# kessel/dune-pnp

Hardware: AMD Instinct MI355X
Metric: assembled DOFs/s + BiCGStab iters/s, 3-species PNP on pore.msh-refined (higher is better)
Workload: dtype f64; 1 GPU; config 3: stationary 3-ion PNP, test/pore_pnp/pore.msh refined k=4 x 1 mirrored copies; dofs=2214099, dofs_per_gpu=2214099, mesh_vertices=738033, triangles=1470464, parallelism=mesh partition (RCB) x1, preconditioner=ilu0, colors=4, sell_slots=5176768, blocks=5155025

## Files before the change

### dune-pnp_amd/csrc/assemble.hip

```cpp
#include <cstdlib>

#include <hip/hip_ext.h>

#include "element.h"
#include "kernels.h"

namespace pnp {

namespace {

template <int OP, int KC = 0>
__device__ __forceinline__ void store_block(double *__restrict__ vc, int lane, int s,
                                            const double *Kc) {
  constexpr int NK = OpTraits<OP>::NK;
  static_assert(!KC || OP == OP_PNP, "constant planes: the PNP operator only");
  constexpr int Q0 = KC ? 2 : 0;
#ifdef ASM_STORE_PLAIN
  store_vals<NK, Q0>(vc + size_t(s) * NK * kRows, lane, Kc);
#else
  store_vals_nt<NK, Q0>(vc + size_t(s) * NK * kRows, lane, Kc);
#endif
}

template <int NF>
// ... 136 lines not shown
      for (int v = 0; v < NK; v++) F[v] += P[v];
      store_block<OP>(vc, lane, 1, F);
    }
    store_block<OP>(vc, lane, 0, D);
  }
  residual_tail<NF>(a, row, a.rowflag[row], R);
}

#ifndef ASM_SU
#define ASM_SU 4
#endif
template <int OP>
__host__ __device__ constexpr int asm_lds_rec() {
  return 2 + OpTraits<OP>::NF + (OP == OP_DIFF || OP == OP_DIFF_IE || OP == OP_POISSON) +
         (OP == OP_POISSON);
}
template <int OP>
constexpr int asm_kc() {
  return OP == OP_PNP;
}
constexpr int kPipeDw = 11;
template <class P>
__device__ __forceinline__ void lds_dma4(const P *src, uint32_t *dst_wave) {
  __builtin_amdgcn_global_load_lds(
      (const __attribute__((address_space(1))) void *)(src),
      (__attribute__((address_space(3))) void *)(dst_wave), 4, 0, 0);
}
__device__ __forceinline__ int const_ld(const int *p, int i) {
  return ((const __attribute__((address_space(4))) int *)(p))[i];
}
__device__ __forceinline__ int row_block_const(const DevLayout &L, int b, int nwg) {
  return L.blkmap ? const_ld(L.blkmap, xcd_block(b, nwg, 1)) : xcd_block(b, nwg, L.xcd_remap);
}
template <int OP, int JAC, int MINW, int FANR, int SPLIT = FANR, int STAGE = 0, int LDSG = 0,
          int KC = 0, int PIPE = 0>
__global__ __launch_bounds__(256, MINW) void k_assemble_ga(DevLayout L, AsmArgs a) {
  using T = OpTraits<OP>;
  constexpr int NF = T::NF, NK = T::NK, NS = FANR;
  constexpr bool AUX0 = OP == OP_DIFF || OP == OP_DIFF_IE || OP == OP_POISSON;
  constexpr bool AUX1 = OP == OP_POISSON;
  constexpr int RW = asm_lds_rec<OP>();
  static_assert(!PIPE || (JAC && FANR == 9 && !STAGE && !LDSG), "PIPE: the direct Jacobian walk");
  extern __shared__ double srec[];
  __shared__ uint32_t pfb[PIPE ? 4 * kPipeDw * kRows : 1];
  const int ntiles = (L.n_owned + 255) / 256, G = gridDim.x;
  const int wv = PIPE ? __builtin_amdgcn_readfirstlane(int(threadIdx.x) / kRows) : 0;
  const int ln = int(threadIdx.x) % kRows;
  uint32_t *const pw = pfb + (PIPE ? wv * kPipeDw * kRows : 0);
  int tile = blockIdx.x, b0 = -1, b1 = -1, b2 = -1, o0 = 0, o1 = 0, c1 = 0;
  auto tile_blk = [&](int t) { return t < ntiles ? row_block_const(L, t, ntiles) : -1; };
  auto wave_chunk = [&](int b) {
    return (b >= 0 && b * 256 + wv * kRows < L.n_owned) ? b * 4 + wv : -1;
  };
  auto prefetch = [&](int b, int off, int clen) {
    if (wave_chunk(b) < 0) return;
    const int r0 = b * 256 + wv * kRows;
    const int *cix = L.colidx + off + ln;
#pragma unroll
    for (int k = 1; k < NS; k++)
      lds_dma4(cix + (k < clen ? k : 0) * kRows, pw + (k - 1) * kRows);
    const uint32_t *m =
        reinterpret_cast<const uint32_t *>(L.rowmeta + min(r0 + ln, L.n_owned - 1));
    lds_dma4(m, pw + 8 * kRows);
    lds_dma4(m + 1, pw + 9 * kRows);
    lds_dma4(reinterpret_cast<const uint32_t *>(a.rowflag + r0) + (ln >> 2), pw + 10 * kRows);
  };
  if constexpr (PIPE) {
    if (tile >= ntiles) return;
    b0 = tile_blk(tile);
    b1 = tile_blk(tile + G);
    b2 = tile_blk(tile + 2 * G);
    int c0 = 0;
    if (wave_chunk(b0) >= 0) {
      o0 = const_ld(L.chunk_off, wave_chunk(b0));
      c0 = const_ld(L.chunk_len, wave_chunk(b0));
    }
    if (wave_chunk(b1) >= 0) {
      o1 = const_ld(L.chunk_off, wave_chunk(b1));
      c1 = const_ld(L.chunk_len, wave_chunk(b1));
    }
    prefetch(b0, o0, c0);
  }
  int o2 = 0, c2 = 0, b3 = -1;
  const auto advance = [&]() {
    tile += G;
    b0 = b1, o0 = o1;
    b1 = b2, o1 = o2, c1 = c2;
    b2 = b3;
    return b0 >= 0;
  };
  do {
    const int blk = PIPE ? b0 : row_block(L, blockIdx.x, gridDim.x);
    const int row0 = blk * blockDim.x + threadIdx.x;
    const bool live = row0 < L.n_owned;
    if (!PIPE && !LDSG && !live) return;
    const int row = live ? row0 : 0;
    const int chunk = row / kRows, lane = row % kRows;
    int cj[NS];
    uint64_t meta_pf = 0;
    unsigned fl_pf = 0;
    if constexpr (PIPE) {
      asm volatile("s_waitcnt vmcnt(0)" ::: "memory");
#pragma unroll
      for (int k = 1; k < NS; k++) cj[k] = int(pw[(k - 1) * kRows + ln]);
      meta_pf = uint64_t(pw[8 * kRows + ln]) | (uint64_t(pw[9 * kRows + ln]) << 32);
      fl_pf = (pw[10 * kRows + ln] >> (8 * (ln & 3))) & 0xffu;
      asm volatile("s_waitcnt lgkmcnt(0)" ::: "memory");
      prefetch(b1, o1, c1);
      o2 = c2 = 0;
      if (wave_chunk(b2) >= 0) {
        o2 = const_ld(L.chunk_off, wave_chunk(b2));
        c2 = const_ld(L.chunk_len, wave_chunk(b2));
      }
      b3 = tile_blk(tile + 3 * G);
      if (!live) continue;
    }
    const int off = PIPE ? o0 : L.chunk_off[chunk];
    const uint64_t meta = PIPE ? meta_pf : L.rowmeta[row];
    const int len = int(meta & 63);
    const bool closed = (meta >> 6) & 1;
    const unsigned brk = unsigned(meta >> 8);
    double *__restrict__ vc = a.vals + size_t(off) * NK;

    if constexpr (PIPE) {
    } else if constexpr (LDSG) {
      const uint16_t *__restrict__ lix = L.lidx + off + lane;
#pragma unroll
      for (int k = 1; k < NS; k++) {
        const int t = lix[(k < len ? k : 0) * kRows];
        cj[k] = k < len ? t : 0;
// ... 125 lines not shown
          double Ct[NK];
#pragma unroll
          for (int v = 0; v < NK; v++) Ct[v] = 0;
          element<OP, JAC, KC>(a, G, pi2.y, pn[s].y, pt.y, ui, un[s], ut, ai, a0[s], at0, aq,
                               a1[s], at1, R, D, P, Ct);
          if constexpr (JAC) {
            if (s == 1 && closed) {
#pragma unroll
              for (int v = 0; v < NK; v++) F[v] = P[v];
            } else {
              put(s, P);
            }
#pragma unroll
            for (int v = 0; v < NK; v++) P[v] = Ct[v];
          }
        } else if constexpr (JAC) {
          put(s, P);
#pragma unroll
          for (int v = 0; v < NK; v++) P[v] = 0;
        }
      }
    }
    if constexpr (JAC) {
      if (closed) {
#pragma unroll
        for (int v = 0; v < NK; v++) F[v] += P[v];
        store_block<OP, KC>(vc, lane, 1, F);
      }
      store_block<OP, KC>(vc, lane, 0, D);
    }
    residual_tail<NF>(a, row, PIPE ? fl_pf : unsigned(a.rowflag[row]), R);
  } while (PIPE && advance());
}

template <int OP>
__global__ __launch_bounds__(256) void k_mass_apply(DevLayout L, double tau, double pi, int cyl,
                                                    const double *__restrict__ xo,
                                                    double *__restrict__ cvec) {
  constexpr int NF = OpTraits<OP>::NF;
  const int row = blockIdx.x * blockDim.x + threadIdx.x;
  if (row >= L.n_owned) return;
  const int chunk = row / kRows, lane = row % kRows;
  const int off = L.chunk_off[chunk];
  const uint64_t meta = L.rowmeta[row];
  const int len = int(meta & 63);
  const bool closed = (meta >> 6) & 1;
  const int *cix = L.colidx + off + lane;
  const double2 pi2 = reinterpret_cast<const double2 *>(L.xy)[row];
  double acc = 0;
  for (int s = 1; s < len; ++s) {
    const int t = (s + 1 < len) ? s + 1 : (closed ? 1 : -1);
    if (t < 0 || ((meta >> (8 + s)) & 1)) continue;
    const int b = cix[s * kRows], c = cix[t * kRows];
    const double2 pb2 = reinterpret_cast<const double2 *>(L.xy)[b];
    const double2 pc2 = reinterpret_cast<const double2 *>(L.xy)[c];
    Geo G;
    geometry(pi2.x, pi2.y, pb2.x, pb2.y, pc2.x, pc2.y, G);
    if constexpr (OP == OP_PNP_IE) {
      double Mii, Mib, Mic;
      mass_q2(G, cyl, pi, pi2.y, pb2.y, pc2.y, Mii, Mib, Mic);
      acc += tau * ((xo[size_t(row) * 3 + 1] + xo[size_t(row) * 3 + 2]) * Mii +
                    (xo[size_t(b) * 3 + 1] + xo[size_t(b) * 3 + 2]) * Mib +
                    (xo[size_t(c) * 3 + 1] + xo[size_t(c) * 3 + 2]) * Mic);
    } else {
      acc += xo[row] * G.adet * (1.0 / 12.0) + (xo[b] + xo[c]) * G.adet * (1.0 / 24.0);
    }
// ... 23 lines not shown
                 uo = x[size_t(q.z) * 3 + f];
    gf[f][0] = ua * G.gi0 + uc * G.gb0 + uo * G.gc0;
    gf[f][1] = ua * G.gi1 + uc * G.gb1 + uo * G.gc1;
  }
  const double cp = 0.5 * (x[size_t(q.x) * 3 + 1] + x[size_t(q.y) * 3 + 1]);
  const double cm = 0.5 * (x[size_t(q.x) * 3 + 2] + x[size_t(q.y) * 3 + 2]);
  const double tx = pc.x - pa.x, ty = pc.y - pa.y;
  const double len = sqrt(tx * tx + ty * ty);
  double factor = len;
  if (cyl) factor *= 2 * pi * (0.5 * (pa.y + pc.y));
  double nx = ty / len, ny = -tx / len;
  if (nx * (po.x - pa.x) + ny * (po.y - pa.y) > 0) {
    nx = -nx;
    ny = -ny;
  }
  const double gp0 = factor * gf[0][0] * cp, gp1 = factor * gf[0][1] * cp;
  out[2 * size_t(k)] = (-factor * gf[1][0] + gp0) * nx + (-factor * gf[1][1] + gp1) * ny;
  const double r = cm / cp;
  out[2 * size_t(k) + 1] =
      (-factor * gf[2][0] - gp0 * r) * nx + (-factor * gf[2][1] - gp1 * r) * ny;
}

}

hipError_t launch_ion_flux(int ns, const int4 *seg, const double *xy, const double *x, int cyl,
                           double pi, double *out, hipStream_t s) {
  if (ns == 0) return hipSuccess;
  hipLaunchKernelGGL(k_ion_flux, dim3((ns + 255) / 256), dim3(256), 0, s, ns, seg, xy, x, cyl, pi,
                     out);
  return hipGetLastError();
}

constexpr bool kAsmPipeDefault = false;

template <int OP>
static int launch_pipe(const DevLayout &L, const AsmArgs &a, int cap, hipStream_t s, hipEvent_t t0,
                       hipEvent_t t1) {
  if constexpr (asm_kc<OP>()) {
    const auto kern = k_assemble_ga<OP, 1, 3, 9, 6, 0, 0, 1, 1>;
    static const int resident = [&] {
      int dev = 0, cus = 0, per_cu = 0;
      if (hipGetDevice(&dev) != hipSuccess ||
          hipDeviceGetAttribute(&cus, hipDeviceAttributeMultiprocessorCount, dev) != hipSuccess ||
          hipOccupancyMaxActiveBlocksPerMultiprocessor(&per_cu, kern, 256, 0) != hipSuccess)
        return 0;
      return per_cu * cus;
    }();
    const int ntiles = (L.n_owned + 255) / 256;
    int g = resident >= 8 ? resident / 8 * 8 : 8;
    if (g > ntiles) g = ntiles;
    if (cap > 0 && g > cap) g = cap;
    hipExtLaunchKernelGGL(kern, dim3(g), dim3(256), 0, s, t0, t1, 0, L, a);
    return 1;
  } else {
    return 0;
  }
}

hipError_t launch_assemble(const DevLayout &L, const AsmArgs &a, hipStream_t s, hipEvent_t t0,
                           hipEvent_t t1, int *pipelined) {
  if (pipelined) *pipelined = 0;
  if (L.n_owned == 0) return hipSuccess;
  dim3 grid((L.n_owned + 255) / 256), block(256);
  static const int waves = [] {
    const char *e = getenv("PNP_ASM_WAVES");
    return (e && atoi(e) == 4) ? 4 : 3;
  }();
  static const bool fanr_ok = [] {
    const char *e = getenv("PNP_ASM_FANR");
    return !(e && atoi(e) == 0);
  }();
  static const int ga = [] {
    const char *e = getenv("PNP_ASM_GA");
    return e ? atoi(e) : 4;
  }();
  const int fanr = !fanr_ok ? 0 : (L.max_slots <= 9 ? 9 : (L.max_slots <= 12 ? 12 : 0));
  static const int lds_env = [] {
    const char *e = getenv("PNP_ASM_LDS");
    return e ? (atoi(e) == 1 ? 1 : 0) : -1;
  }();
  static const bool cold_hint = [] {
    const char *e = getenv("PNP_ASM_COLD_HINT");
    return !(e && e[0] == '0');
  }();
  const auto lds_walk = [&](int nk) {
    return lds_env == 1 ||
           (lds_env < 0 && (size_t(L.n_owned) * 7 * size_t(nk) * 8 > (size_t(512) << 20) ||
                            (cold_hint && a.cold)));
  };
  static const bool pipe_on = [] {
    const char *e = getenv("PNP_ASM_PIPE");
    return e ? atoi(e) != 0 : kAsmPipeDefault;
  }();
  static const int pipe_cap = [] {
    const char *e = getenv("PNP_ASM_PIPE_GRID");
    return (e && atoi(e) >= 1) ? atoi(e) : 0;
  }();
  int piped = 0;
#define PNP_ASM_CASE(OPK)                                                          \
  case OPK:                                                                        \
    if (!fanr && a.jac)                                                            \
      hipExtLaunchKernelGGL((k_assemble<OPK, 1, 3, 0>), grid, block, 0, s, t0, t1, 0, L, a);     \
    else if (!fanr)                                                                \
      hipExtLaunchKernelGGL((k_assemble<OPK, 0, 4, 0>), grid, block, 0, s, t0, t1, 0, L, a);     \
    else if (!a.jac && fanr == 9 && ga && lds_env == 1 && L.uown &&                 \
             size_t(L.unmax) * asm_lds_rec<OPK>() * 8 <= 53 * 1024)                    \
      hipExtLaunchKernelGGL((k_assemble_ga<OPK, 0, 3, 9, 9, 0, 1>), grid, block,         \
                         size_t(L.unmax) * asm_lds_rec<OPK>() * 8, s, t0, t1, 0, L, a);             \
    else if (!a.jac && fanr == 9 && ga)                                            \
      hipExtLaunchKernelGGL((k_assemble_ga<OPK, 0, 3, 9>), grid, block, 0, s, t0, t1, 0, L, a);  \
    else if (!a.jac)                                                               \
      hipExtLaunchKernelGGL((k_assemble<OPK, 0, 4, 12>), grid, block, 0, s, t0, t1, 0, L, a);    \
    else if (ga == 1 && fanr == 9)                                                 \
      hipExtLaunchKernelGGL((k_assemble_ga<OPK, 1, 3, 9>), grid, block, 0, s, t0, t1, 0, L, a);  \
    else if (ga == 2 && fanr == 9)                                                 \
      hipExtLaunchKernelGGL((k_assemble_ga<OPK, 1, 2, 9>), grid, block, 0, s, t0, t1, 0, L, a);  \
    else if (ga == 3 && fanr == 9)                                                 \
      hipExtLaunchKernelGGL((k_assemble_ga<OPK, 1, 3, 9, 5>), grid, block, 0, s, t0, t1, 0, L, a); \
    else if (ga == 4 && fanr == 9 && asm_kc<OPK>() && a.kconst &&                   \
             lds_walk(OpTraits<OPK>::NK) && L.uown &&                               \
             size_t(L.unmax) * asm_lds_rec<OPK>() * 8 <= 53 * 1024)                    \
      hipExtLaunchKernelGGL((k_assemble_ga<OPK, 1, 3, 9, 6, 0, 1, asm_kc<OPK>()>), grid,  \
                         block, size_t(L.unmax) * asm_lds_rec<OPK>() * 8, s, t0, t1, 0, L, a); \
    else if (ga == 4 && fanr == 9 && asm_kc<OPK>() && a.kconst && pipe_on)         \
      piped = launch_pipe<OPK>(L, a, pipe_cap, s, t0, t1);                         \
    else if (ga == 4 && fanr == 9 && asm_kc<OPK>() && a.kconst)                    \
      hipExtLaunchKernelGGL((k_assemble_ga<OPK, 1, 3, 9, 6, 0, 0, asm_kc<OPK>()>), grid,  \
                         block, 0, s, t0, t1, 0, L, a);                             \
    else if (ga == 4 && fanr == 9 && lds_walk(OpTraits<OPK>::NK) && L.uown &&       \
             size_t(L.unmax) * asm_lds_rec<OPK>() * 8 <= 53 * 1024)                    \
      hipExtLaunchKernelGGL((k_assemble_ga<OPK, 1, 3, 9, 6, 0, 1>), grid, block,         \
                         size_t(L.unmax) * asm_lds_rec<OPK>() * 8, s, t0, t1, 0, L, a);             \
    else if (ga == 4 && fanr == 9)                                                 \
      hipExtLaunchKernelGGL((k_assemble_ga<OPK, 1, 3, 9, 6>), grid, block, 0, s, t0, t1, 0, L, a); \
    else if (ga == 5 && fanr == 9)                                                 \
      hipExtLaunchKernelGGL((k_assemble_ga<OPK, 1, 3, 9, 3>), grid, block, 0, s, t0, t1, 0, L, a); \
    else if (ga == 6 && fanr == 9)                                                 \
      hipExtLaunchKernelGGL((k_assemble_ga<OPK, 1, 3, 9, 6, 1>), grid, block, 0, s, t0, t1, 0, L, a); \
    else if (fanr == 12)                                                           \
      hipExtLaunchKernelGGL((k_assemble<OPK, 1, 3, 12>), grid, block, 0, s, t0, t1, 0, L, a);    \
    else if (waves == 3)                                                           \
      hipExtLaunchKernelGGL((k_assemble<OPK, 1, 3, 9>), grid, block, 0, s, t0, t1, 0, L, a);     \
    else                                                                           \
      hipExtLaunchKernelGGL((k_assemble<OPK, 1, 4, 9>), grid, block, 0, s, t0, t1, 0, L, a);     \
    break;
  switch (a.kind) {
    PNP_ASM_CASE(OP_PNP)
    PNP_ASM_CASE(OP_PNP_IE)
    PNP_ASM_CASE(OP_PB)
    PNP_ASM_CASE(OP_DIFF)
    PNP_ASM_CASE(OP_DIFF_IE)
    PNP_ASM_CASE(OP_POISSON)
  default:
    return hipErrorInvalidValue;
  }
#undef PNP_ASM_CASE
  if (pipelined) *pipelined = piped;
  return hipGetLastError();
// ... 19 lines not shown
```

### dune-pnp_amd/csrc/ctx.cc

```cpp
#include "ctx.h"

static thread_local std::string g_err;
std::mutex g_groups_m;
std::map<std::string, std::shared_ptr<LocalGroup>> g_groups;

void pnp_ctx::asm_wrote(bool kc, bool full) {
  if (kc) {
    asm_reused++;
  } else {
    asm_full++;
    vals_const_valid = full;
  }
}

pnp_ctx::~pnp_ctx() {
  graphs_clear();
  for (auto &v : ev_pending)
    for (auto &pr : v) {
      hipEventDestroy(pr.first);
      hipEventDestroy(pr.second);
    }
  for (auto e : ev_pool) hipEventDestroy(e);
  if (hS) hipHostFree(hS);
  if (h_send) hipHostFree(h_send);
// ... 2882 lines not shown

extern "C" int pnp_idr_info(pnp_ctx *c, int64_t *replacements) {
  if (!c) return PNP_E_ARG;
  if (replacements) *replacements = c->idr_replacements;
  return PNP_OK;
}

extern "C" int pnp_idr_shadow(pnp_ctx *c, int32_t j, double *p) {
  if (!c || !p) return PNP_E_ARG;
  if (!c->idr_P.p || c->idr_P_s != c->idr_s || c->idr_P_nf != c->nf)
    return c->fail(PNP_E_STATE, "no IDR solve yet with the current PNP_OPT_IDR_S and operator");
  if (j < 0 || j >= c->idr_s) return c->fail(PNP_E_ARG, "shadow column out of range");
  hipSetDevice(c->device);
  return c->download_ext(c->idr_P.p + size_t(j) * size_t(c->idr_ld(false)), c->nf, p);
}

extern "C" int pnp_asm_row_flags(pnp_ctx *c, uint8_t *flags) {
  if (!c || !flags) return PNP_E_ARG;
  if (c->kind < 0) return c->fail(PNP_E_STATE, "no operator set (pnp_set_operator)");
  if (c->degree > 1) return c->fail(PNP_E_STATE, "row flags: P1 contexts only");
  std::memset(flags, 0xff, size_t(c->mesh.nv));
  for (int i = 0; i < c->L.n_owned; i++) flags[c->L.l2g[i]] = c->hrowflag[i];
  return PNP_OK;
}

extern "C" int pnp_asm_info(pnp_ctx *c, int64_t *full, int64_t *reused, int64_t *pipelined) {
  if (!c) return PNP_E_ARG;
  if (full) *full = c->asm_full;
  if (reused) *reused = c->asm_reused;
  if (pipelined) *pipelined = c->asm_piped;
  return PNP_OK;
}

extern "C" int pnp_amg_configure(pnp_ctx *c, const pnp_amg_opts *o) {
  if (!c || !o) return PNP_E_ARG;
  if (o->smoother != PNP_PREC_SSOR && o->smoother != PNP_PREC_ILU0 &&
      o->smoother != PNP_PREC_JACOBI && o->smoother != PNP_PREC_SSOR_NATURAL)
    return c->fail(PNP_E_ARG, "AMG smoother must be SSOR, SSOR_NATURAL, ILU0 or JACOBI");
  if (o->coarse_target < 1 || o->coarse_target > pnp::kAmgMaxCoarse || o->max_levels < 2 ||
      o->max_levels > pnp::kAmgMaxLevels || !(o->omega > 0 && o->omega <= 2) ||
      o->coarse_sweeps < 1 || o->coarse_sweeps > 8 || o->level0_presmooth < -1 ||
      o->level0_presmooth > 1)
    return c->fail(PNP_E_ARG, "AMG options out of range");
  const bool rebuild = o->coarse_target != c->amg_opts.coarse_target ||
                       o->max_levels != c->amg_opts.max_levels;
  c->amg_opts = *o;
  if (rebuild) c->amg_built = false;
  c->amg_values_drop();
  return PNP_OK;
}

extern "C" int pnp_amg_info(pnp_ctx *c, pnp_amg_stats *st) {
  if (!c || !st) return PNP_E_ARG;
  std::memset(st, 0, sizeof *st);
  if (!c->amg_built) return c->fail(PNP_E_STATE, "AMG not set up (solve or apply with PNP_PREC_AMG)");
  st->levels = int(c->amg_h.size()) + 1;
  st->rows[0] = c->L.n_owned;
  st->blocks[0] = c->L.nblocks;
  for (size_t k = 0; k < c->amg_h.size() && k + 1 < 16; k++) {
    st->rows[k + 1] = c->amg_h[k].nb;
    st->blocks[k + 1] = (int64_t)c->amg_h[k].col.size();
  }
  st->omega = c->amg_opts.omega;
  st->smoother = c->amg_opts.smoother;
  return PNP_OK;
}
// ... 374 lines not shown
}

extern "C" int pnp_space(pnp_ctx *c, pnp_space_info *info, double *xy, int32_t *enode) {
  if (!c || !info) return PNP_E_ARG;
  const bool pk = c->degree > 1;
  info->degree = c->degree;
  info->nnodes = c->mesh.nv;
  info->nt = pk ? c->tmesh.nt : c->mesh.nt;
  info->nlocal = pk ? c->pks.nl : 3;
  if (xy) std::memcpy(xy, c->mesh.xy.data(), sizeof(double) * c->mesh.xy.size());
  if (enode) {
    const std::vector<int> &en = pk ? c->pks.enode : c->mesh.tri;
    std::memcpy(enode, en.data(), sizeof(int) * en.size());
  }
  return PNP_OK;
}

extern "C" int pnp_state_set(pnp_ctx *c, const double *x) {
  if (!c || !x) return PNP_E_ARG;
  if (c->kind < 0) return c->fail(PNP_E_STATE, "no operator set");
  hipSetDevice(c->device);
  int rc = c->upload_ext(x, c->nf, c->x.p, true);
  if (rc) return rc;
  CK(hipStreamSynchronize(c->stream), "state_set");
  return PNP_OK;
}

extern "C" int pnp_state_get(pnp_ctx *c, double *x) {
  if (!c || !x) return PNP_E_ARG;
  hipSetDevice(c->device);
  return c->download_ext(c->x.p, c->nf, x);
}

extern "C" int pnp_assemble_state(pnp_ctx *c, int32_t n) {
  if (!c) return PNP_E_ARG;
  hipSetDevice(c->device);
  const int jac = n >= 0 ? 1 : 0;
  for (int k = 0; k < (n >= 0 ? n : -n); k++) {
    int rc = c->assemble(c->x.p, jac);
    if (rc) return rc;
  }
  CK(hipStreamSynchronize(c->stream), "assemble_state");
  return PNP_OK;
}

extern "C" int pnp_assemble_state_timed(pnp_ctx *c, int32_t n, double *ms) {
  if (!c || !ms || n == 0) return PNP_E_ARG;
  hipSetDevice(c->device);
  const bool timing = c->timing;
  c->timing = false;
  hipEvent_t e0 = c->ev_get(), e1 = c->ev_get();
  hipEventRecord(e0, c->stream);
  int rc = PNP_OK;
  for (int k = 0; k < (n >= 0 ? n : -n) && rc == PNP_OK; k++) rc = c->assemble(c->x.p, n >= 0);
  hipEventRecord(e1, c->stream);
  c->timing = timing;
  const hipError_t e = hipStreamSynchronize(c->stream);
  float t = 0;
  if (rc == PNP_OK && e == hipSuccess) hipEventElapsedTime(&t, e0, e1);
  c->ev_pool.push_back(e0);
  c->ev_pool.push_back(e1);
  if (rc) return rc;
  CK(e, "assemble_state_timed");
  *ms = t;
  return PNP_OK;
}
// ... 196 lines not shown
    return PNP_E_MESH;
  }
  *out = b.release();
  return PNP_OK;
}

extern "C" int pnp_layout_view(const pnp_layout_buf *b, pnp_layout *v) {
  if (!b || !v) return PNP_E_ARG;
  const pnp::LocalLayout &L = b->L;
  v->n_owned = L.n_owned;
  v->n_ghost = L.n_ghost;
  v->ncolors = int(L.color_ptr.size()) - 1;
  v->nchunks = L.nchunks;
  v->nnbr = int(L.nbr_ranks.size());
  v->max_slots = b->fans.max_slots;
  v->nslots = L.nslots;
  v->nblocks = L.nblocks;
  v->l2g = L.l2g.data();
  v->color_ptr = L.color_ptr.data();
  v->color_idx = L.color_idx.data();
  v->rowcolor = L.rowcolor.data();
  v->chunk_len = L.chunk_len.data();
  v->chunk_off = L.chunk_off.data();
  v->colidx = L.colidx.data();
  v->rowmeta = L.rowmeta.data();
  v->nbr_ranks = L.nbr_ranks.data();
  v->recv_ptr = L.recv_ptr.data();
  v->send_ptr = L.send_ptr.data();
  v->send_idx = L.send_idx.data();
  v->color_conflicts = L.conflicts;
  return PNP_OK;
}

extern "C" void pnp_layout_free(pnp_layout_buf *b) { delete b; }
```

### dune-pnp_amd/csrc/mesh.h

```cpp
#pragma once

#include <atomic>

#include <array>
#include <cstdint>
#include <map>
#include <string>
#include <vector>

namespace pnp {

struct Mesh {
  int nv = 0, nt = 0, nb = 0;
  std::vector<double> xy;
  std::vector<int> tri;
  std::vector<int> bseg;
  std::vector<int> bgroup;
};

bool read_gmsh(const std::string &path, Mesh &m, std::string &err);
bool write_gmsh(const std::string &path, const Mesh &m, std::string &err);
Mesh refine(const Mesh &m, int k);
bool validate(const Mesh &m, std::string &err);

struct GeoModel {
  std::map<int, std::array<double, 3>> pts;
  struct Curve {
    bool circle = false;
    int a = -1, b = -1, c = -1;
  };
  std::map<int, Curve> curves;
  std::map<int, std::vector<int>> loops;
  std::map<int, std::vector<int>> surfaces;
  std::map<int, int> curve_group;
// ... 25 lines not shown
  std::vector<Surface> surf;
};

void dirichlet_mask(const Mesh &m, const Params &p, int nf, int field0, std::vector<uint8_t> &mask);
void neumann_load(const Mesh &m, const Params &p, int nf, int field0, std::vector<double> &load);
void initial_state(const Mesh &m, const Params &p, const double *phi_pb, double *x0);
void initial_state_at(const Mesh &m, const Params &p, int nl, const int *enode, const double *nxy,
                      int nn, const double *phi_pb, double *x0);

void rcb_partition(const Mesh &m, int nparts, std::vector<int> &part);

constexpr int kChunk = 64;
constexpr int kOrderBlock = 4096;

struct LocalLayout {
  int rank = 0, nranks = 1;
  int n_owned = 0, n_ghost = 0;
  std::vector<int> l2g;
  std::vector<int> g2l;
  std::vector<int> color_ptr, color_idx;
  std::vector<uint8_t> rowcolor;
  int nchunks = 0;
  std::vector<int> chunk_len, chunk_off;
  std::vector<int> colidx;
  std::vector<uint64_t> rowmeta;
  std::vector<int> xmap;
  long long nslots = 0;
  long long nblocks = 0;
  long long conflicts = 0;
  std::vector<int> nbr_ranks;
  std::vector<int> recv_ptr, send_ptr, send_idx;
};

extern std::atomic<int> g_absorb_thin_color;
bool build_local_layout(const Mesh &m, const Fans &f, const std::vector<int> &part, int rank,
                        int nranks, LocalLayout &L, std::string &err);

}
```

### dune-pnp_amd/python/pnp_amd/__init__.py

```python
from __future__ import annotations

import ctypes as C
import os
from dataclasses import dataclass

import numpy as np

HERE = os.path.dirname(os.path.abspath(__file__))
PKG_ROOT = os.path.dirname(os.path.dirname(HERE))
REPO_ROOT = os.path.dirname(PKG_ROOT)
LIB_PATH = os.environ.get("PNP_AMD_LIB") or os.path.join(PKG_ROOT, "libpnp_amd.so")
HEADER = os.path.join(REPO_ROOT, "include", "pnp_capi.h")

OK, E_ARG, E_HIP, E_RCCL, E_BREAKDOWN, E_NOT_CONVERGED, E_IO, E_MESH, E_STATE = \
    0, -1, -2, -3, -4, -5, -6, -7, -8
OP_PNP, OP_PNP_IMPLICIT_EULER, OP_PB, OP_DIFF, OP_DIFF_IMPLICIT_EULER, OP_POISSON = range(6)
PREC_NONE, PREC_SSOR, PREC_ILU0, PREC_JACOBI, PREC_AMG, PREC_SSOR_NATURAL = range(6)
METHOD_BICGSTAB, METHOD_CG, METHOD_GMRES, METHOD_FGMRES, METHOD_IDR = 0, 1, 2, 3, 4
(OPT_ILU_F32, OPT_ILU_FUSED_FACTOR, OPT_JAC_FD, OPT_BICG_TWORED, OPT_AMG_FALLBACK,
 OPT_GRAPH, OPT_SEQ_ORDER, OPT_ILU_FLOW, OPT_NAT_FLOW, OPT_ILU_RETRY,
 OPT_GMRES_RESTART, OPT_MATRIX_FREE, OPT_ASM_REUSE_CONST, OPT_IDR_S) = (1, 2, 3, 4, 5, 6, 7, 8,
                                                                        9, 10, 11, 12, 13, 14)
ASM_PIPE_ENV, ASM_PIPE_GRID_ENV = "PNP_ASM_PIPE", "PNP_ASM_PIPE_GRID"
ROW_FLAG_LOAD = 8
DEVICE_PTRS, JAC_FD = 1, 2
CREATE_ABSORB_THIN_COLOR = 1
PREC_BY_NAME = {"none": PREC_NONE, "nonprec": PREC_NONE, "ssor": PREC_SSOR, "ilu0": PREC_ILU0,
                "jacobi": PREC_JACOBI, "amg": PREC_AMG, "ssor_natural": PREC_SSOR_NATURAL}
MAX_SURFACES = 64


class PnpError(RuntimeError):
    def __init__(self, code, msg):
        super().__init__(f"pnp error {code}: {msg}")
        self.code = code


class _Mesh(C.Structure):
    _fields_ = [("nv", C.c_int32), ("coords", C.c_void_p), ("nt", C.c_int32),
                ("tri", C.c_void_p), ("nbseg", C.c_int32), ("bseg", C.c_void_p),
                ("bseg_group", C.c_void_p)]


class _Surface(C.Structure):
    _fields_ = [("coulomb_btype", C.c_int32), ("coulomb_flux", C.c_double),
                ("coulomb_potential", C.c_double), ("plus_btype", C.c_int32),
                ("plus_flux", C.c_double), ("plus_concentration", C.c_double),
                ("minus_btype", C.c_int32), ("minus_flux", C.c_double),
                ("minus_concentration", C.c_double)]


class _Params(C.Structure):
    _fields_ = [("l_b", C.c_double), ("c0", C.c_double), ("tau", C.c_double), ("pi", C.c_double),
                ("cylindrical", C.c_int32), ("n_surfaces", C.c_int32), ("surfaces", C.c_void_p)]


# ... 373 lines not shown
    x0 = np.zeros(3 * mesh.nv)
    m = mesh.c()
    _check(lib().pnp_setup_initial_state(C.byref(m), C.byref(params.c), _ptr(phi), _ptr(x0)))
    return x0


class Layout:

    def __init__(self, mesh: Mesh, rank=0, nranks=1):
        buf = C.c_void_p()
        m = mesh.c()
        _check(lib().pnp_layout_build(C.byref(m), int(rank), int(nranks), C.byref(buf)))
        v = _Layout()
        _check(lib().pnp_layout_view(buf, C.byref(v)))

        def arr(p, n, dt=np.int32):
            return np.ctypeslib.as_array(p, (n,)).astype(dt).copy() if n else np.zeros(0, dt)
        self.n_owned, self.n_ghost = v.n_owned, v.n_ghost
        self.ncolors, self.nchunks, self.max_slots = v.ncolors, v.nchunks, v.max_slots
        self.nslots, self.nblocks = v.nslots, v.nblocks
        self.l2g = arr(v.l2g, v.n_owned + v.n_ghost)
        self.color_ptr = arr(v.color_ptr, v.ncolors + 1)
        self.color_idx = arr(v.color_idx, v.n_owned)
        self.rowcolor = arr(v.rowcolor, v.n_owned + v.n_ghost, np.uint8)
        self.chunk_len = arr(v.chunk_len, v.nchunks)
        self.chunk_off = arr(v.chunk_off, v.nchunks + 1)
        self.colidx = arr(v.colidx, v.nslots)
        self.rowmeta = arr(v.rowmeta, v.n_owned, np.uint64)
        self.nbr_ranks = arr(v.nbr_ranks, v.nnbr)
        self.recv_ptr = arr(v.recv_ptr, v.nnbr + 1)
        self.send_ptr = arr(v.send_ptr, v.nnbr + 1)
        self.send_idx = arr(v.send_idx, int(self.send_ptr[-1]) if v.nnbr else 0)
        self.color_conflicts = int(v.color_conflicts)
        lib().pnp_layout_free(buf)

    def row_len(self, i):
        return int(self.rowmeta[i] & np.uint64(63))

    def row_cols(self, i):
        c, lane = divmod(i, 64)
        L = self.row_len(i)
        return [int(self.colidx[self.chunk_off[c] + s * 64 + lane]) for s in range(L)]


def set_create_option(option, value):
    _check(lib().pnp_set_create_option(option, C.c_int64(value)))


def get_create_option(option):
    v = C.c_int64(0)
    _check(lib().pnp_get_create_option(option, C.byref(v)))
    return v.value


def rccl_unique_id() -> bytes:
    buf = C.create_string_buffer(128)
    _check(lib().pnp_rccl_unique_id(buf))
    return buf.raw


class Context:

    def __init__(self, mesh: Mesh, params: Params, device=0, rank=0, size=1, unique_id=None,
                 local_group=None, degree=1, host_transport=None):
        self.mesh, self.params = mesh, params
        self._uid = C.create_string_buffer(unique_id, 128) if unique_id else None
# ... 234 lines not shown
        out = C.c_double(0)
        self._ck(lib().pnp_norm(self.h, _ptr(a), nfields or (a.size // self.nn), 0, C.byref(out)))
        return out.value

    def newton_history(self):
        n = C.c_int32(0)
        self._ck(lib().pnp_newton_history(self.h, None, None, 0, C.byref(n)))
        its = np.zeros(n.value, dtype=np.int32)
        dfs = np.zeros(n.value)
        self._ck(lib().pnp_newton_history(self.h, _ptr(its), _ptr(dfs), n.value, C.byref(n)))
        return its, dfs

    def sync_vector(self, v, nfields=None):
        nf = nfields or (v.size // self.nn)
        v = np.ascontiguousarray(v, dtype=np.float64).copy()
        self._ck(lib().pnp_sync_vector(self.h, _ptr(v), int(nf)))
        return v

    def initial_state(self, phi_pb):
        phi = np.ascontiguousarray(phi_pb, dtype=np.float64)
        x0 = np.zeros(3 * self.nn)
        self._ck(lib().pnp_initial_state(self.h, _ptr(phi), _ptr(x0)))
        return x0

    def state_set(self, x):
        x = self._vec(x)
        self._ck(lib().pnp_state_set(self.h, _ptr(x)))

    def state_get(self):
        x = np.zeros(self.nf * self.nn)
        self._ck(lib().pnp_state_get(self.h, _ptr(x)))
        return x

    def assemble_state(self, n=1):
        self._ck(lib().pnp_assemble_state(self.h, int(n)))

    def assemble_state_timed(self, n=1):
        ms = C.c_double()
        self._ck(lib().pnp_assemble_state_timed(self.h, int(n), C.byref(ms)))
        return ms.value / 1e3

    def bicgstab_iterations(self, n, prec=PREC_NONE):
        r = _SolveResult()
        self._ck(lib().pnp_bicgstab_iterations(self.h, int(n), int(prec), C.byref(r)))
        return {k: getattr(r, k) for k, _ in _SolveResult._fields_}

    def set_option(self, option, value):
        self._ck(lib().pnp_set_option(self.h, int(option), C.c_int64(int(value))))

    def get_option(self, option):
        v = C.c_int64()
        self._ck(lib().pnp_get_option(self.h, int(option), C.byref(v)))
        return v.value

    def matfree_info(self):
        a, v = C.c_int64(), C.c_int64()
        self._ck(lib().pnp_matfree_info(self.h, C.byref(a), C.byref(v)))
        return {"applies": a.value, "value_assemblies": v.value}

    def asm_info(self):
        f, r, p = C.c_int64(), C.c_int64(), C.c_int64()
        self._ck(lib().pnp_asm_info(self.h, C.byref(f), C.byref(r), C.byref(p)))
        return {"full": f.value, "reused": r.value, "pipelined": p.value}

    def asm_row_flags(self):
        out = np.zeros(self.mesh.nv, dtype=np.uint8)
        self._ck(lib().pnp_asm_row_flags(self.h, out.ctypes.data_as(C.c_void_p)))
        return out

    def probe_slot_stores(self, tile_elems=256, reps=20):
        o = _StoreProbe()
        self._ck(lib().pnp_probe_slot_stores(self.h, int(tile_elems), int(reps), C.byref(o)))
        return {k: getattr(o, k) for k, _ in _StoreProbe._fields_}

    def cache_scrub(self, nbytes=1 << 30):
        self._ck(lib().pnp_cache_scrub(self.h, C.c_int64(int(nbytes))))

    def timers(self, enable=None, reset=False):
        if enable is not None:
            self._ck(lib().pnp_timers_enable(self.h, int(bool(enable))))
        if reset:
            self._ck(lib().pnp_timers_reset(self.h))
        t = _Timers()
        self._ck(lib().pnp_timers_get(self.h, C.byref(t)))
        return {k: getattr(t, k) for k, _ in _Timers._fields_}


def header_symbols():
    import re
    txt = open(HEADER).read()
    return sorted(set(re.findall(r"^\s*(?:int|void|const char \*)\s*(pnp_\w+)\s*\(", txt, re.M)))


def header_constants():
    import re
    txt = open(HEADER).read()
# ... 2 lines not shown
```

### include/pnp_capi.h

```cpp
#ifndef PNP_CAPI_H
#define PNP_CAPI_H

#include <stdint.h>

#ifdef __cplusplus
extern "C" {
#endif

#define PNP_CAPI_VERSION 1

enum {
  PNP_OK = 0,
  PNP_E_ARG = -1,
  PNP_E_HIP = -2,
  PNP_E_RCCL = -3,
  PNP_E_BREAKDOWN = -4,
  PNP_E_NOT_CONVERGED = -5,
  PNP_E_IO = -6,
  PNP_E_MESH = -7,
  PNP_E_STATE = -8
};

typedef struct pnp_ctx pnp_ctx;

// ... 171 lines not shown
  double omega;
  int32_t coarse_sweeps;
  int32_t level0_presmooth;
} pnp_amg_opts;
int pnp_amg_configure(pnp_ctx *ctx, const pnp_amg_opts *opts);
typedef struct {
  int32_t levels;
  int32_t smoother;
  int32_t rows[16];
  int64_t blocks[16];
  double omega;
} pnp_amg_stats;
int pnp_amg_info(pnp_ctx *ctx, pnp_amg_stats *stats);
int pnp_amg_aggregates(pnp_ctx *ctx, int32_t level, int32_t *agg);

enum {
  PNP_OPT_ILU_F32 = 1,
  PNP_OPT_ILU_FUSED_FACTOR = 2,
  PNP_OPT_JAC_FD = 3,
  PNP_OPT_BICG_TWORED = 4,
  PNP_OPT_AMG_FALLBACK = 5,
  PNP_OPT_GRAPH = 6,
  PNP_OPT_SEQ_ORDER = 7,
  PNP_OPT_ILU_FLOW = 8,
  PNP_OPT_NAT_FLOW = 9,
  PNP_OPT_ILU_RETRY = 10,
  PNP_OPT_GMRES_RESTART = 11,
  PNP_OPT_MATRIX_FREE = 12,
  PNP_OPT_ASM_REUSE_CONST = 13,
  PNP_OPT_IDR_S = 14
};
int pnp_set_option(pnp_ctx *ctx, int32_t option, int64_t value);
int pnp_asm_info(pnp_ctx *ctx, int64_t *full, int64_t *reused, int64_t *pipelined);
#define PNP_ROW_FLAG_LOAD 8
int pnp_asm_row_flags(pnp_ctx *ctx, uint8_t *flags);
int pnp_matfree_info(pnp_ctx *ctx, int64_t *applies, int64_t *value_assemblies);
int pnp_idr_info(pnp_ctx *ctx, int64_t *replacements);
int pnp_idr_shadow(pnp_ctx *ctx, int32_t j, double *p);

enum {
  PNP_CREATE_ABSORB_THIN_COLOR = 1
};
int pnp_set_create_option(int32_t option, int64_t value);
int pnp_get_create_option(int32_t option, int64_t *value);
int pnp_get_option(pnp_ctx *ctx, int32_t option, int64_t *value);

int pnp_linear_solve(pnp_ctx *ctx, const double *rhs, double *z, const pnp_solve_opts *opts,
                     pnp_solve_result *res);
int pnp_linear_solve_ex(pnp_ctx *ctx, const double *rhs, double *z, const pnp_solve_opts *opts,
                        pnp_solve_result *res, int32_t flags);

int pnp_solve_history(pnp_ctx *ctx, double *defects, int32_t cap, int32_t *n);

typedef struct {
  double reduction, abs_limit, min_linear_reduction;
  int32_t maxit, line_search_maxit;
  pnp_solve_opts linear;
} pnp_newton_opts;
typedef struct {
  int32_t converged, iterations, linear_iterations, status;
  double first_defect, defect, elapsed, assemble_seconds, solve_seconds;
  int32_t linear_fallbacks;
  int32_t precision_retries;
} pnp_newton_result;
int pnp_newton(pnp_ctx *ctx, double *u, const pnp_newton_opts *opts, pnp_newton_result *res);
int pnp_newton_history(pnp_ctx *ctx, int32_t *linear_iterations, double *defects, int32_t cap,
                       int32_t *nsteps);

int pnp_sync_vector(pnp_ctx *ctx, double *v, int32_t nfields);

int pnp_dot(pnp_ctx *ctx, const double *a, const double *b, int32_t nfields, int32_t flags,
            double *out);
int pnp_norm(pnp_ctx *ctx, const double *a, int32_t nfields, int32_t flags, double *out);

int pnp_initial_state(pnp_ctx *ctx, const double *phi_pb, double *x0);

int pnp_ion_flux(pnp_ctx *ctx, const double *x, int32_t nsurf, double *ip, double *im);

typedef struct {
  double dt, t0;
  int32_t nsteps, potential_update_freq, output_freq;
  double red_diffusion, red_poisson;
  pnp_solve_opts linear;
  int32_t reuse;
} pnp_md_opts;
typedef struct {
  int32_t status, steps_done;
  int32_t diffusion_solves, poisson_solves, linear_iterations;
  int32_t assemblies, prec_setups;
  int32_t noutputs;
  double elapsed;
} pnp_md_result;
int pnp_md_run(pnp_ctx *ctx, double *u, const pnp_md_opts *opts, int32_t nsurf, int32_t cap,
               double *t_out, double *ip, double *im, pnp_md_result *res, int32_t flags);

int pnp_state_set(pnp_ctx *ctx, const double *x);
int pnp_state_get(pnp_ctx *ctx, double *x);
int pnp_assemble_state(pnp_ctx *ctx, int32_t n);
int pnp_assemble_state_timed(pnp_ctx *ctx, int32_t n, double *ms);
int pnp_bicgstab_iterations(pnp_ctx *ctx, int32_t n, int32_t prec, pnp_solve_result *res);

typedef struct {
  double us_sell, us_tile, us_tile_sorted, us_random;
  int64_t slot_bytes;
  int64_t rows, rows_whole, tiles, elements;
} pnp_store_probe;
int pnp_probe_slot_stores(pnp_ctx *ctx, int32_t tile_elems, int32_t reps, pnp_store_probe *out);

int pnp_cache_scrub(pnp_ctx *ctx, int64_t bytes);

typedef struct {
  double assemble_ms, spmv_ms, prec_ms, blas_ms, halo_ms, allreduce_ms;
  int64_t assemble_launches, spmv_launches, prec_launches, blas_launches;
  double factor_ms;
  int64_t factor_launches;
} pnp_timers;
int pnp_timers_enable(pnp_ctx *ctx, int32_t on);
int pnp_timers_get(pnp_ctx *ctx, pnp_timers *t);
int pnp_timers_reset(pnp_ctx *ctx);


int pnp_setup_boundary(const pnp_mesh *mesh, const pnp_params *params, int32_t nfields,
                       int32_t field0, uint8_t *mask, double *load);
int pnp_setup_initial_state(const pnp_mesh *mesh, const pnp_params *params, const double *phi_pb,
                            double *x0);

typedef struct pnp_layout_buf pnp_layout_buf;
typedef struct {
  int32_t n_owned, n_ghost, ncolors, nchunks, nnbr, max_slots;
  int64_t nslots, nblocks;
  const int32_t *l2g;
  const int32_t *color_ptr;
  const int32_t *color_idx;
  const uint8_t *rowcolor;
  const int32_t *chunk_len;
  const int32_t *chunk_off;
  const int32_t *colidx;
  const uint64_t *rowmeta;
  const int32_t *nbr_ranks;
  const int32_t *recv_ptr;
  const int32_t *send_ptr;
  const int32_t *send_idx;
  int64_t color_conflicts;
} pnp_layout;
int pnp_layout_build(const pnp_mesh *mesh, int32_t rank, int32_t nranks, pnp_layout_buf **out);
int pnp_layout_view(const pnp_layout_buf *b, pnp_layout *view);
void pnp_layout_free(pnp_layout_buf *b);

#ifdef __cplusplus
}
#endif
#endif
```

Before: 53.27 billion assembled DOFs/s.

## Add fully unrolled fast path for regular 6-neighbour interior rows in PNP assembly

Adds a REG variant of the direct constant-planes Jacobian assembly kernel. When every row in a wave has exactly six closed-fan neighbours and no boundary metadata, it takes a specialised path that is unrolled over a compile-time slot count, gathers neighbour coordinates and state into registers up front, and uses uniform residual handling. This removes the variable-length loop, per-slot branching and metadata lookups for the common interior case, at the cost of higher register pressure and a ballot-based fallback when a wave is mixed. It is enabled by default through PNP_ASM_REGULAR, and the change also adds diagnostics APIs that count regular chunks and expose the residual.

```diff
diff --git a/dune-pnp_amd/csrc/assemble.hip b/dune-pnp_amd/csrc/assemble.hip
--- a/dune-pnp_amd/csrc/assemble.hip
+++ b/dune-pnp_amd/csrc/assemble.hip
@@ -192,8 +192,13 @@
 __device__ __forceinline__ int row_block_const(const DevLayout &L, int b, int nwg) {
   return L.blkmap ? const_ld(L.blkmap, xcd_block(b, nwg, 1)) : xcd_block(b, nwg, L.xcd_remap);
 }
+template <int OP>
+constexpr int asm_reg() {
+  return OP == OP_PNP;
+}
+constexpr int kRegSlots = 7;
 template <int OP, int JAC, int MINW, int FANR, int SPLIT = FANR, int STAGE = 0, int LDSG = 0,
-          int KC = 0, int PIPE = 0>
+          int KC = 0, int PIPE = 0, int REG = 0>
 __global__ __launch_bounds__(256, MINW) void k_assemble_ga(DevLayout L, AsmArgs a) {
   using T = OpTraits<OP>;
   constexpr int NF = T::NF, NK = T::NK, NS = FANR;
@@ -201,6 +206,8 @@
   constexpr bool AUX1 = OP == OP_POISSON;
   constexpr int RW = asm_lds_rec<OP>();
   static_assert(!PIPE || (JAC && FANR == 9 && !STAGE && !LDSG), "PIPE: the direct Jacobian walk");
+  static_assert(!REG || (OP == OP_PNP && JAC && KC && FANR == 9 && !STAGE && !LDSG && !PIPE),
+                "REG: OP_PNP, the direct constant-planes Jacobian walk");
   extern __shared__ double srec[];
   __shared__ uint32_t pfb[PIPE ? 4 * kPipeDw * kRows : 1];
   const int ntiles = (L.n_owned + 255) / 256, G = gridDim.x;
@@ -256,6 +263,86 @@
     if (!PIPE && !LDSG && !live) return;
     const int row = live ? row0 : 0;
     const int chunk = row / kRows, lane = row % kRows;
+    if constexpr (REG) {
+      const uint64_t meta = L.rowmeta[row];
+      const bool regular =
+          int(meta & 63) == kRegSlots && ((meta >> 6) & 1) && (meta >> 8) == 0;
+      if (__all(regular)) {
+        const int off = L.chunk_off[chunk];
+        const int *__restrict__ cix = L.colidx + off + lane;
+        int cr[kRegSlots];
+#pragma unroll
+        for (int k = 1; k < kRegSlots; k++) cr[k] = cix[k * kRows];
+        const unsigned fl = a.rowflag[row];
+        const double2 pi2 = reinterpret_cast<const double2 *>(L.xy)[row];
+        double ui[NF];
+        load_nf<NF>(a.x, size_t(row), ui);
+        double2 pn[kRegSlots];
+        double un[kRegSlots][NF];
+        auto gather = [&](int k) {
+          pn[k] = reinterpret_cast<const double2 *>(L.xy)[cr[k]];
+          load_nf<NF>(a.x, size_t(cr[k]), un[k]);
+        };
+#pragma unroll
+        for (int k = 1; k < kRegSlots - 1; k++) gather(k);
+        double *__restrict__ vc = a.vals + size_t(off) * NK;
+        double R[NF], D[NK], P[NK], F[NK];
+#pragma unroll
+        for (int f = 0; f < NF; f++) R[f] = 0;
+#pragma unroll
+        for (int v = 0; v < NK; v++) D[v] = P[v] = F[v] = 0;
+#pragma unroll
+        for (int s = 1; s < kRegSlots; s++) {
+          const int t = s + 1 < kRegSlots ? s + 1 : 1;
+          double2 pt = pn[t], ps = pn[s];
+          double ut[NF], us[NF];
+          asm volatile("" : "+v"(pt.x), "+v"(pt.y));
+#pragma unroll
+          for (int f = 0; f < NF; f++) {
+            ut[f] = un[t][f];
+            asm volatile("" : "+v"(ut[f]));
+          }
+          asm volatile("" : "+v"(ps.x), "+v"(ps.y));
+#pragma unroll
+          for (int f = 0; f < NF; f++) {
+            us[f] = un[s][f];
+            asm volatile("" : "+v"(us[f]));
+          }
+          Geo G;
+          geometry(pi2.x, pi2.y, ps.x, ps.y, pt.x, pt.y, G);
+          double Ct[NK];
+#pragma unroll
+          for (int v = 0; v < NK; v++) Ct[v] = 0;
+          element<OP, JAC, KC>(a, G, pi2.y, ps.y, pt.y, ui, us, ut, 0.0, 0.0, 0.0, 0.0, 0.0, 0.0, R,
+                               D, P, Ct);
+          if (s == 1) {
+#pragma unroll
+            for (int v = 0; v < NK; v++) F[v] = P[v];
+          } else {
+            if (s == 2) gather(kRegSlots - 1);
+            store_block<OP, KC>(vc, lane, s, P);
+          }
+#pragma unroll
+          for (int v = 0; v < NK; v++) P[v] = Ct[v];
+#pragma unroll
+          for (int f = 0; f < NF; f++) asm volatile("" : "+v"(R[f]));
+#pragma unroll
+          for (int v = 2; v < NK; v++) asm volatile("" : "+v"(D[v]));
+        }
+#pragma unroll
+        for (int v = 0; v < NK; v++) F[v] += P[v];
+        store_block<OP, KC>(vc, lane, 1, F);
+        store_block<OP, KC>(vc, lane, 0, D);
+        if (__any(fl & kRowFlagLoad))
+          residual_tail<NF>(a, row, fl, R);
+        else
+          residual_tail<NF>(a, row, fl & ~unsigned(kRowFlagLoad), R);
+        return;
+      }
+#ifdef ASM_REGULAR_CHECK
+      return;
+#endif
+    }
     int cj[NS];
     uint64_t meta_pf = 0;
     unsigned fl_pf = 0;
@@ -447,6 +534,10 @@
     residual_tail<NF>(a, row, PIPE ? fl_pf : unsigned(a.rowflag[row]), R);
   } while (PIPE && advance());
 }
+
+#ifdef ASM_REGULAR_CHECK
+template __global__ void k_assemble_ga<OP_PNP, 1, 3, 7, 7, 0, 0, 1>(DevLayout, AsmArgs);
+#endif
 
 template <int OP>
 __global__ __launch_bounds__(256) void k_mass_apply(DevLayout L, double tau, double pi, int cyl,
@@ -536,6 +627,7 @@
 }
 
 constexpr bool kAsmPipeDefault = false;
+constexpr bool kAsmRegularDefault = true;
 
 template <int OP>
 static int launch_pipe(const DevLayout &L, const AsmArgs &a, int cap, hipStream_t s, hipEvent_t t0,
@@ -600,6 +692,10 @@
     const char *e = getenv("PNP_ASM_PIPE_GRID");
     return (e && atoi(e) >= 1) ? atoi(e) : 0;
   }();
+  static const bool regular_on = [] {
+    const char *e = getenv("PNP_ASM_REGULAR");
+    return e ? atoi(e) != 0 : kAsmRegularDefault;
+  }();
   int piped = 0;
 #define PNP_ASM_CASE(OPK)                                                          \
   case OPK:                                                                        \
@@ -628,6 +724,10 @@
                          block, size_t(L.unmax) * asm_lds_rec<OPK>() * 8, s, t0, t1, 0, L, a); \
     else if (ga == 4 && fanr == 9 && asm_kc<OPK>() && a.kconst && pipe_on)         \
       piped = launch_pipe<OPK>(L, a, pipe_cap, s, t0, t1);                         \
+    else if (ga == 4 && fanr == 9 && asm_kc<OPK>() && a.kconst && regular_on)      \
+      hipExtLaunchKernelGGL(                                                       \
+          (k_assemble_ga<OPK, 1, 3, 9, 6, 0, 0, asm_kc<OPK>(), 0, asm_reg<OPK>()>), grid, block, \
+          0, s, t0, t1, 0, L, a);                                                  \
     else if (ga == 4 && fanr == 9 && asm_kc<OPK>() && a.kconst)                    \
       hipExtLaunchKernelGGL((k_assemble_ga<OPK, 1, 3, 9, 6, 0, 0, asm_kc<OPK>()>), grid,  \
                          block, 0, s, t0, t1, 0, L, a);                             \
diff --git a/dune-pnp_amd/csrc/ctx.cc b/dune-pnp_amd/csrc/ctx.cc
--- a/dune-pnp_amd/csrc/ctx.cc
+++ b/dune-pnp_amd/csrc/ctx.cc
@@ -2938,6 +2938,15 @@
   return PNP_OK;
 }
 
+extern "C" int pnp_asm_regular_info(pnp_ctx *c, int64_t *chunks, int64_t *regular_chunks) {
+  if (!c) return PNP_E_ARG;
+  long long n = 0, r = 0;
+  pnp::regular_chunks(c->L, n, r);
+  if (chunks) *chunks = n;
+  if (regular_chunks) *regular_chunks = r;
+  return PNP_OK;
+}
+
 extern "C" int pnp_amg_configure(pnp_ctx *c, const pnp_amg_opts *o) {
   if (!c || !o) return PNP_E_ARG;
   if (o->smoother != PNP_PREC_SSOR && o->smoother != PNP_PREC_ILU0 &&
@@ -3378,6 +3387,15 @@
   return c->download_ext(c->x.p, c->nf, x);
 }
 
+extern "C" int pnp_state_residual(pnp_ctx *c, double *r) {
+  if (!c || !r) return PNP_E_ARG;
+  if (c->kind < 0) return c->fail(PNP_E_STATE, "no operator set");
+  if (c->seq_on() || c->degree > 1)
+    return c->fail(PNP_E_STATE, "pnp_state_residual: P1 contexts, not in reference-order mode");
+  hipSetDevice(c->device);
+  return c->download_ext(c->r.p, c->nf, r);
+}
+
 extern "C" int pnp_assemble_state(pnp_ctx *c, int32_t n) {
   if (!c) return PNP_E_ARG;
   hipSetDevice(c->device);
@@ -3640,4 +3658,14 @@
   return PNP_OK;
 }
 
+extern "C" int pnp_layout_regular_info(const pnp_layout_buf *b, int64_t *chunks,
+                                       int64_t *regular_chunks) {
+  if (!b) return PNP_E_ARG;
+  long long n = 0, r = 0;
+  pnp::regular_chunks(b->L, n, r);
+  if (chunks) *chunks = n;
+  if (regular_chunks) *regular_chunks = r;
+  return PNP_OK;
+}
+
 extern "C" void pnp_layout_free(pnp_layout_buf *b) { delete b; }
diff --git a/dune-pnp_amd/csrc/mesh.h b/dune-pnp_amd/csrc/mesh.h
--- a/dune-pnp_amd/csrc/mesh.h
+++ b/dune-pnp_amd/csrc/mesh.h
@@ -1,5 +1,6 @@
 #pragma once
 
+#include <algorithm>
 #include <atomic>
 
 #include <array>
@@ -91,6 +92,20 @@
   std::vector<int> recv_ptr, send_ptr, send_idx;
 };
 
+static inline bool meta_regular(uint64_t m) {
+  return meta_len(m) == 7 && meta_closed(m) && (m >> 8) == 0;
+}
+static inline void regular_chunks(const LocalLayout &L, long long &chunks, long long &regular) {
+  chunks = L.nchunks;
+  regular = 0;
+  for (int c = 0; c < L.nchunks; c++) {
+    bool all = true;
+    for (int i = c * kChunk; i < std::min((c + 1) * kChunk, L.n_owned) && all; i++)
+      all = meta_regular(L.rowmeta[i]);
+    regular += all;
+  }
+}
+
 extern std::atomic<int> g_absorb_thin_color;
 bool build_local_layout(const Mesh &m, const Fans &f, const std::vector<int> &part, int rank,
                         int nranks, LocalLayout &L, std::string &err);
diff --git a/dune-pnp_amd/python/pnp_amd/__init__.py b/dune-pnp_amd/python/pnp_amd/__init__.py
--- a/dune-pnp_amd/python/pnp_amd/__init__.py
+++ b/dune-pnp_amd/python/pnp_amd/__init__.py
@@ -22,6 +22,7 @@
  OPT_GMRES_RESTART, OPT_MATRIX_FREE, OPT_ASM_REUSE_CONST, OPT_IDR_S) = (1, 2, 3, 4, 5, 6, 7, 8,
                                                                         9, 10, 11, 12, 13, 14)
 ASM_PIPE_ENV, ASM_PIPE_GRID_ENV = "PNP_ASM_PIPE", "PNP_ASM_PIPE_GRID"
+ASM_REGULAR_ENV = "PNP_ASM_REGULAR"
 ROW_FLAG_LOAD = 8
 DEVICE_PTRS, JAC_FD = 1, 2
 CREATE_ABSORB_THIN_COLOR = 1
@@ -461,6 +462,9 @@
         self.send_ptr = arr(v.send_ptr, v.nnbr + 1)
         self.send_idx = arr(v.send_idx, int(self.send_ptr[-1]) if v.nnbr else 0)
         self.color_conflicts = int(v.color_conflicts)
+        n, r = C.c_int64(0), C.c_int64(0)
+        _check(lib().pnp_layout_regular_info(buf, C.byref(n), C.byref(r)))
+        self.regular_info = {"chunks": n.value, "regular_chunks": r.value}
         lib().pnp_layout_free(buf)
 
     def row_len(self, i):
@@ -761,6 +765,11 @@
         self._ck(lib().pnp_state_get(self.h, _ptr(x)))
         return x
 
+    def state_residual(self):
+        r = np.zeros(self.nf * self.nn)
+        self._ck(lib().pnp_state_residual(self.h, _ptr(r)))
+        return r
+
     def assemble_state(self, n=1):
         self._ck(lib().pnp_assemble_state(self.h, int(n)))
 
@@ -791,6 +800,11 @@
         f, r, p = C.c_int64(), C.c_int64(), C.c_int64()
         self._ck(lib().pnp_asm_info(self.h, C.byref(f), C.byref(r), C.byref(p)))
         return {"full": f.value, "reused": r.value, "pipelined": p.value}
+
+    def asm_regular_info(self):
+        n, r = C.c_int64(0), C.c_int64(0)
+        self._ck(lib().pnp_asm_regular_info(self.h, C.byref(n), C.byref(r)))
+        return {"chunks": n.value, "regular_chunks": r.value}
 
     def asm_row_flags(self):
         out = np.zeros(self.mesh.nv, dtype=np.uint8)
diff --git a/include/pnp_capi.h b/include/pnp_capi.h
--- a/include/pnp_capi.h
+++ b/include/pnp_capi.h
@@ -227,6 +227,7 @@
 };
 int pnp_set_option(pnp_ctx *ctx, int32_t option, int64_t value);
 int pnp_asm_info(pnp_ctx *ctx, int64_t *full, int64_t *reused, int64_t *pipelined);
+int pnp_asm_regular_info(pnp_ctx *ctx, int64_t *chunks, int64_t *regular_chunks);
 #define PNP_ROW_FLAG_LOAD 8
 int pnp_asm_row_flags(pnp_ctx *ctx, uint8_t *flags);
 int pnp_matfree_info(pnp_ctx *ctx, int64_t *applies, int64_t *value_assemblies);
@@ -291,6 +292,7 @@
 
 int pnp_state_set(pnp_ctx *ctx, const double *x);
 int pnp_state_get(pnp_ctx *ctx, double *x);
+int pnp_state_residual(pnp_ctx *ctx, double *r);
 int pnp_assemble_state(pnp_ctx *ctx, int32_t n);
 int pnp_assemble_state_timed(pnp_ctx *ctx, int32_t n, double *ms);
 int pnp_bicgstab_iterations(pnp_ctx *ctx, int32_t n, int32_t prec, pnp_solve_result *res);
@@ -340,6 +342,7 @@
 } pnp_layout;
 int pnp_layout_build(const pnp_mesh *mesh, int32_t rank, int32_t nranks, pnp_layout_buf **out);
 int pnp_layout_view(const pnp_layout_buf *b, pnp_layout *view);
+int pnp_layout_regular_info(const pnp_layout_buf *b, int64_t *chunks, int64_t *regular_chunks);
 void pnp_layout_free(pnp_layout_buf *b);
 
 #ifdef __cplusplus
```

After: 56.23 billion assembled DOFs/s (median of 6 runs). +5.6%, better.
